# equinor/gordo

Measured on AMD Instinct MI355X. Metric: machines built/hour (1000-model config), higher is better.
Workload: dtype bf16; 1 GPU; global_batch=125, machines_per_gpu=125, seq_len=144, rows=4320, n_tags=50, epochs=5, parallelism=fleet-dp1 (RCCL shard, grouped MFMA packs per rank)

## Files before the change

### gordo_amd/ops/__init__.py

```python
from .api import (
    ACT_LINEAR,
    ACT_TANH,
    ACT_RELU,
    ACT_SIGMOID,
    act_code,
    hip_available,
    grouped_linear_fwd,
    act_l1_bwd,
    grouped_linear_bwd_data,
    grouped_linear_wgrad,
    grouped_gemm_acc,
    mse_bwd,
    adam_step,
    loss_bwd,
    optimizer_step,
    masked_copy,
    segment_table,
    lstm_pointwise_fwd,
    lstm_seq_fwd,
    lstm_seq_fwd_v3,
    lstm_seq_fwd_v2,
    lstm_seq_bwd,
    lstm_seq_bwd_v2,
    last_scan_launch,
    last_scan_activation,
    lstm_act_scan_available,
    last_wgrad_launch,
    lstm_seq_bwd_v3,
    lstm_seq_available,
    lstm_v4_available,
    lstm_seq_fwd_fused,
    lstm_seq_bwd_fused,
    lstm_seq_bwd_fused_out,
    lstm_seq_bwd_v3_out,
    anomaly_score,
    trail_min_max,
    grouped_linear_wgrad_hprev,
    window_gather,
    grouped_wgrad_xh,
    windowed_quantile,
    row_quantile,
    lstm_pointwise_bwd,
)

__all__ = [
    "ACT_LINEAR",
    "ACT_TANH",
    "ACT_RELU",
    "ACT_SIGMOID",
    "act_code",
    "hip_available",
    "grouped_linear_fwd",
    "act_l1_bwd",
    "grouped_linear_bwd_data",
    "grouped_linear_wgrad",
    "grouped_gemm_acc",
    "mse_bwd",
    "adam_step",
    "loss_bwd",
    "optimizer_step",
    "masked_copy",
    "segment_table",
    "lstm_pointwise_fwd",
    "lstm_seq_fwd",
    "lstm_seq_fwd_v3",
    "lstm_seq_fwd_v2",
    "lstm_seq_bwd",
    "lstm_seq_bwd_v2",
    "last_scan_launch",
    "last_scan_activation",
    "lstm_act_scan_available",
    "last_wgrad_launch",
    "lstm_seq_bwd_v3",
    "trail_min_max",
    "grouped_linear_wgrad_hprev",
    "window_gather",
    "grouped_wgrad_xh",
    "windowed_quantile",
    "row_quantile",
    "lstm_seq_available",
    "lstm_v4_available",
    "lstm_seq_fwd_fused",
    "lstm_seq_bwd_fused",
    "lstm_seq_bwd_fused_out",
    "lstm_seq_bwd_v3_out",
    "anomaly_score",
    "lstm_pointwise_bwd",
]
```

### gordo_amd/ops/api.py

```python
from __future__ import annotations

from typing import Optional, Tuple

import torch

from . import reference as ref
from .reference import (
    ACT_LINEAR,
    ACT_TANH,
    ACT_RELU,
    ACT_SIGMOID,
    act_code,
)

_hip = None
_hip_err: Optional[str] = None


def _load_hip():
    global _hip, _hip_err
    if _hip is not None or _hip_err is not None:
        return _hip
    try:
        from . import _gordo_hip
# ... 168 lines not shown
    elif kind == "rmsprop":
        code = _OPT_RMSPROP
        vals = [lr, h["rho"], h["momentum"], h["epsilon"]]
    elif kind == "adagrad":
        code, vals = _OPT_ADAGRAD, [lr, h["epsilon"], 0.0, 0.0]
    elif kind == "adam":
        code = _OPT_ADAM_AMSGRAD
        vals = [lr, h["beta_1"], h["beta_2"], h["epsilon"]]
    elif kind == "adamax":
        code = _OPT_ADAMAX
        vals = [lr, h["beta_1"], h["beta_2"], h["epsilon"]]
    else:
        raise ValueError(f"Unsupported optimizer {kind!r}")
    if active is not None:
        return _require_hip().optimizer_step_masked(
            code, p, g, s0, s1, s2, [float(v) for v in vals], flag, p_lp,
            step_buf, active, segments,
        )
    return _require_hip().optimizer_step(
        code, p, g, s0, s1, s2, [float(v) for v in vals], flag, p_lp,
        step_buf,
    )


def lstm_seq_fwd(xW, Wh):
    import os as _os

    ext = _require_hip()
    G, B = xW.shape[0], xW.shape[1]
    H = xW.shape[-1] // 4
    v2_fills = H % 16 == 0 and G * ((B + 63) // 64) >= 256
    if (
        _os.environ.get("GORDO_LSTM_V1") == "1"
        or H > 64
        or v2_fills
    ):
        return ext.lstm_seq_fwd(xW, Wh)
    return ext.lstm_seq_fwd_v3(xW, Wh)


def lstm_v4_available(H: int, F: int) -> bool:
    return hip_available() and H <= 64 and H % 8 == 0 and F % 8 == 0 \
        and F <= 128


def lstm_act_scan_available(H: int, F: int) -> bool:
    import os as _os

    return (
        lstm_v4_available(H, F)
        and F >= 8
        and _os.environ.get("GORDO_LSTM_V4", "1") != "0"
        and _os.environ.get("GORDO_LSTM_PIPE", "1") != "0"
    )


def lstm_seq_fwd_fused(xseq, Wx, Wh, bias, store_aux=True, act="tanh"):
    act = act_code(act)
    if _on_gpu(xseq):
        return _require_hip().lstm_seq_fwd_fused(
            xseq, Wx, Wh, bias, bool(store_aux), act
        )
    G, B, T, F = xseq.shape
    H = Wh.shape[1]
    gates_all = ref.grouped_linear_fwd(
        xseq.reshape(G, B * T, F), Wx, bias, ACT_LINEAR
    ).view(G, B, T, 4 * H)
    h = torch.zeros(G, B, H, dtype=xseq.dtype)
    c = torch.zeros(G, B, H, dtype=torch.float32)
    hs = torch.empty(G, B, T, H, dtype=xseq.dtype)
    cs = torch.empty(G, B, T, H, dtype=torch.float32)
    ga = torch.empty(G, B, T, 4 * H, dtype=xseq.dtype)
    for t in range(T):
        gates = gates_all[:, :, t] + torch.bmm(h, Wh)
        h, c, gact = ref.lstm_pointwise_fwd(gates, c, act)
        hs[:, :, t] = h
        cs[:, :, t] = c
        ga[:, :, t] = gact
    if store_aux:
        return [hs, cs, ga]
    return [hs]


def lstm_seq_fwd_v3(xW, Wh):
    return _require_hip().lstm_seq_fwd_v3(xW, Wh)


def lstm_seq_fwd_v2(xW, Wh):
    H = xW.shape[-1] // 4
    if H % 16 != 0 or H > 64:
        raise ValueError("lstm_seq_fwd_v2 needs H % 16 == 0 and H <= 64")
    return _require_hip().lstm_seq_fwd(xW, Wh)


def lstm_seq_bwd_v2(dSeq, gacts, cs, Wh, last_only):
    H = gacts.shape[-1] // 4
    if H % 16 != 0 or H > 64:
        raise ValueError("lstm_seq_bwd_v2 needs H % 16 == 0 and H <= 64")
    return _require_hip().lstm_seq_bwd(dSeq, gacts, cs, Wh, bool(last_only))


def last_scan_launch() -> dict:
    family, rows, hf, has_dx, last_only = _require_hip().last_scan_launch()
    return {
        "family": family,
        "rows": rows,
        "hf": hf if hf > 0 else None,
        "has_dx": None if has_dx < 0 else bool(has_dx),
        "last_only": None if last_only < 0 else bool(last_only),
    }


def last_scan_activation() -> str:
    return _require_hip().last_scan_activation()


def lstm_seq_bwd(dSeq, gacts, cs, Wh, last_only, act="tanh"):
    import os as _os

    ext = _require_hip()
    act = act_code(act)
    if act != ACT_TANH:
        return ext.lstm_seq_bwd_v3(dSeq, gacts, cs, Wh, bool(last_only), act)
    G, B = gacts.shape[0], gacts.shape[1]
    H = gacts.shape[-1] // 4
    v2_fills = H % 16 == 0 and G * ((B + 63) // 64) >= 256
    if (
        _os.environ.get("GORDO_LSTM_V1") == "1"
        or H > 64
        or v2_fills
    ):
        return ext.lstm_seq_bwd(dSeq, gacts, cs, Wh, last_only)
    return ext.lstm_seq_bwd_v3(dSeq, gacts, cs, Wh, last_only)


def _lstm_seq_bwd_cpu(dSeq, gacts, cs, Wh, last_only, act):
    G, B, T, H4 = gacts.shape
    H = H4 // 4
    WhT = Wh.transpose(1, 2)
    dh_carry = torch.zeros(G, B, H, dtype=gacts.dtype)
    dc = torch.zeros(G, B, H, dtype=cs.dtype)
    dG = torch.empty_like(gacts)
    zero_c = torch.zeros_like(cs[:, :, 0])
    for t in range(T - 1, -1, -1):
        dh = dh_carry
        if not last_only:
            dh = dh + dSeq[:, :, t]
        elif t == T - 1:
            dh = dh + dSeq
        c_prev = cs[:, :, t - 1] if t > 0 else zero_c
        dg, dc = ref.lstm_pointwise_bwd(
            dh, dc, gacts[:, :, t], cs[:, :, t], c_prev, act
        )
        dG[:, :, t] = dg
        dh_carry = torch.bmm(dg, WhT)
    return dG


def lstm_seq_bwd_fused(dSeq, gacts, cs, Wh, Wx, last_only, act="tanh"):
    act = act_code(act)
    if _on_gpu(gacts):
        out = _require_hip().lstm_seq_bwd_fused(
            dSeq, gacts, cs, Wh, Wx, bool(last_only), act
        )
        return out[0], out[1]
    dG = _lstm_seq_bwd_cpu(dSeq, gacts, cs, Wh, last_only, act)
    G, B, T, H4 = gacts.shape
    dX = ref.grouped_linear_bwd_data(
        dG.view(G, B * T, H4), Wx
    ).view(G, B, T, Wx.shape[1])
    return dG, dX


def lstm_seq_bwd_v3(dSeq, gacts, cs, Wh, last_only, act="tanh"):
    act = act_code(act)
    if not _on_gpu(gacts):
        return _lstm_seq_bwd_cpu(dSeq, gacts, cs, Wh, last_only, act)
    return _require_hip().lstm_seq_bwd_v3(
        dSeq, gacts, cs, Wh, bool(last_only), act
    )


def lstm_seq_bwd_fused_out(dSeq, gacts, cs, Wh, Wx, last_only, dG, dX,
                           act="tanh"):
    _require_hip().lstm_seq_bwd_fused_out(
        dSeq, gacts, cs, Wh, Wx, bool(last_only), dG, dX, act_code(act)
    )


def lstm_seq_bwd_v3_out(dSeq, gacts, cs, Wh, last_only, dG, act="tanh"):
    _require_hip().lstm_seq_bwd_v3_out(
        dSeq, gacts, cs, Wh, bool(last_only), dG, act_code(act)
    )


def lstm_seq_available(H: int) -> bool:
    if not hip_available():
# ... 56 lines not shown
```

### gordo_amd/ops/csrc/gordo_kernels.hip

```cpp

#include <hip/hip_runtime.h>
#include <hip/hip_bf16.h>
#include <torch/extension.h>
#include <ATen/cuda/CUDAContext.h>

#include <cstdint>
#include <cstdlib>
#include <string>
#include <tuple>
#include <vector>

#define DEV_INLINE __device__ __forceinline__

using bf16 = __hip_bfloat16;

typedef __attribute__((ext_vector_type(4))) float f32x4;
typedef __attribute__((ext_vector_type(8))) short bf16x8;

constexpr int ACT_LINEAR = 0, ACT_TANH = 1, ACT_RELU = 2, ACT_SIGMOID = 3;

DEV_INLINE float fast_tanhf(float x);

DEV_INLINE float act_apply(float z, int act) {
  switch (act) {
// ... 716 lines not shown
    switch (act) {                                                          \
      case ACT_LINEAR:                                                      \
        hipLaunchKernelGGL(K<ACT_LINEAR>, __VA_ARGS__); break;              \
      case ACT_RELU:                                                        \
        hipLaunchKernelGGL(K<ACT_RELU>, __VA_ARGS__); break;                \
      case ACT_SIGMOID:                                                     \
        hipLaunchKernelGGL(K<ACT_SIGMOID>, __VA_ARGS__); break;             \
      default:                                                              \
        hipLaunchKernelGGL(K<ACT_TANH>, __VA_ARGS__); break;                \
    }                                                                       \
  } while (0)

std::vector<torch::Tensor> lstm_pointwise_fwd(torch::Tensor gates,
                                              torch::Tensor c_prev,
                                              int64_t act) {
  CHECK_GPU(gates);
  TORCH_CHECK(act >= ACT_LINEAR && act <= ACT_SIGMOID,
              "unknown LSTM cell activation code ", act);
  auto gc = to_bf16c(gates);
  auto cp = c_prev.to(torch::kFloat32).contiguous();
  int H4 = gc.size(-1);
  int H = H4 / 4;
  size_t rows = gc.numel() / H4;
  auto sizes = gc.sizes().vec();
  sizes.back() = H;
  auto h = torch::empty(sizes, gc.options());
  auto c = torch::empty(sizes, gc.options().dtype(torch::kFloat32));
  auto gact = torch::empty_like(gc);
  size_t n = rows * H;
  int blocks = (int)std::min<size_t>((n + 255) / 256, 2048);
  GORDO_CELL_ACT_LAUNCH(lstm_pw_fwd_kernel, dim3(blocks), dim3(256), 0,
                        cur_stream(), (const bf16*)gc.data_ptr(),
                        cp.data_ptr<float>(), (bf16*)h.data_ptr(),
                        c.data_ptr<float>(), (bf16*)gact.data_ptr(), rows, H);
  return {h, c, gact};
}

std::vector<torch::Tensor> lstm_pointwise_bwd(torch::Tensor dh,
                                              torch::Tensor dc_next,
                                              torch::Tensor gact,
                                              torch::Tensor c,
                                              torch::Tensor c_prev,
                                              int64_t act) {
  CHECK_GPU(dh);
  TORCH_CHECK(act >= ACT_LINEAR && act <= ACT_SIGMOID,
              "unknown LSTM cell activation code ", act);
  auto dhc = to_bf16c(dh);
  auto dcn = dc_next.to(torch::kFloat32).contiguous();
  auto gc = to_bf16c(gact);
  auto cc = c.to(torch::kFloat32).contiguous();
  auto cpc = c_prev.to(torch::kFloat32).contiguous();
  int H = dhc.size(-1);
  size_t rows = dhc.numel() / H;
  auto dgates = torch::empty_like(gc);
  auto dc_prev = torch::empty_like(cc);
  size_t n = rows * H;
  int blocks = (int)std::min<size_t>((n + 255) / 256, 2048);
  GORDO_CELL_ACT_LAUNCH(lstm_pw_bwd_kernel, dim3(blocks), dim3(256), 0,
                        cur_stream(), (const bf16*)dhc.data_ptr(),
                        dcn.data_ptr<float>(), (const bf16*)gc.data_ptr(),
                        cc.data_ptr<float>(), cpc.data_ptr<float>(),
                        (bf16*)dgates.data_ptr(), dc_prev.data_ptr<float>(),
                        rows, H);
  return {dgates, dc_prev};
}
#undef GORDO_CELL_ACT_LAUNCH

}

namespace gordo_anomaly {
std::vector<torch::Tensor> anomaly_score(
    torch::Tensor out, torch::Tensor y, torch::Tensor scale,
    torch::Tensor minv, c10::optional<torch::Tensor> feat_thr,
    double agg_thr);
}

namespace gordo_lstm {
std::vector<torch::Tensor> lstm_seq_fwd(torch::Tensor xW, torch::Tensor Wh);
std::vector<torch::Tensor> lstm_seq_fwd_fused(torch::Tensor xseq,
                                              torch::Tensor Wx,
                                              torch::Tensor Wh,
                                              torch::Tensor bias,
                                              bool store_aux, int64_t act);
std::vector<torch::Tensor> lstm_seq_fwd_v3(torch::Tensor xW, torch::Tensor Wh);
torch::Tensor lstm_seq_bwd_v3(torch::Tensor dSeq, torch::Tensor gacts,
                              torch::Tensor cs, torch::Tensor Wh,
                              bool last_only, int64_t act);
std::vector<torch::Tensor> lstm_seq_bwd_fused(
    torch::Tensor dSeq, torch::Tensor gacts, torch::Tensor cs,
    torch::Tensor Wh, torch::Tensor Wx, bool last_only, int64_t act);
torch::Tensor lstm_seq_bwd(torch::Tensor dSeq, torch::Tensor gacts,
                           torch::Tensor cs, torch::Tensor Wh,
                           bool last_only);
void lstm_seq_bwd_fused_out(torch::Tensor dSeq, torch::Tensor gacts,
                            torch::Tensor cs, torch::Tensor Wh,
                            torch::Tensor Wx, bool last_only,
                            torch::Tensor dG, torch::Tensor dX, int64_t act);
void lstm_seq_bwd_v3_out(torch::Tensor dSeq, torch::Tensor gacts,
                         torch::Tensor cs, torch::Tensor Wh, bool last_only,
                         torch::Tensor dG, int64_t act);
std::tuple<std::string, int, int, int, int> last_scan_launch();
std::string last_scan_activation();
}

namespace gordo_thresholds {
torch::Tensor trail_min_max(torch::Tensor X, int64_t w);
torch::Tensor windowed_quantile(torch::Tensor X, int64_t w, double q);
torch::Tensor row_quantile(torch::Tensor X, double q);
}

namespace gordo_train {
std::vector<torch::Tensor> loss_bwd(torch::Tensor Y, torch::Tensor T,
                                    int64_t kind, int64_t real_f,
                                    double delta, bool want_grad);
void optimizer_step(int64_t kind, torch::Tensor p, torch::Tensor g,
                    c10::optional<torch::Tensor> s0,
                    c10::optional<torch::Tensor> s1,
                    c10::optional<torch::Tensor> s2,
                    std::vector<double> hyper, bool flag,
                    c10::optional<torch::Tensor> plp,
                    torch::Tensor step_buf);
}

namespace gordo_masked {
void optimizer_step_masked(int64_t kind, torch::Tensor p, torch::Tensor g,
                           c10::optional<torch::Tensor> s0,
                           c10::optional<torch::Tensor> s1,
                           c10::optional<torch::Tensor> s2,
                           std::vector<double> hyper, bool flag,
                           c10::optional<torch::Tensor> plp,
                           torch::Tensor step_buf, torch::Tensor active,
                           torch::Tensor table);
void masked_copy(torch::Tensor dst, torch::Tensor src, torch::Tensor mask,
                 torch::Tensor table, c10::optional<torch::Tensor> dst_lp);
}

PYBIND11_MODULE(TORCH_EXTENSION_NAME, mod) {
  mod.def("optimizer_step_masked", &gordo_masked::optimizer_step_masked,
          "optimizer step (every kind, plain Adam = 0) over the models "
          "with active[g] != 0 only");
  mod.def("masked_copy", &gordo_masked::masked_copy, py::arg("dst"),
          py::arg("src"), py::arg("mask"), py::arg("table"),
          py::arg("dst_lp") = py::none(),
          "copy the slices of the models with mask[g] != 0 (+ bf16 "
          "mirror)");
  mod.def("loss_bwd", &gordo_train::loss_bwd,
          "fused per-model loss (mse/mae/huber/logcosh) + grad + "
          "accuracy count, one pass over (Y, T)");
  mod.def("optimizer_step", &gordo_train::optimizer_step,
          "fused SGD/RMSprop/Adagrad/Adam-amsgrad/Adamax + bf16 mirror "
          "refresh");
  mod.def("trail_min_max", &gordo_thresholds::trail_min_max,
          "rolling(w).min().max() per row (K10)");
  mod.def("windowed_quantile", &gordo_thresholds::windowed_quantile,
          "rolling(w).quantile(q) per row — q=0.5 is the smm smoothing "
          "(K11)");
  mod.def("row_quantile", &gordo_thresholds::row_quantile,
          "NaN-dropping linear-interpolated quantile per row (K12)");
  mod.def("anomaly_score", &gordo_anomaly::anomaly_score,
          "fused DiffBased anomaly scoring (serving hot path)");
  mod.def("lstm_seq_bwd_v3", &gordo_lstm::lstm_seq_bwd_v3, py::arg("dSeq"),
          py::arg("gacts"), py::arg("cs"), py::arg("Wh"),
          py::arg("last_only"), py::arg("act") = (int64_t)ACT_TANH,
          "pipelined fused LSTM backward scan (GORDO_LSTM_V3 opt-in)");
  mod.def("lstm_seq_fwd_v3", &gordo_lstm::lstm_seq_fwd_v3,
          "pipelined fused LSTM forward scan (GORDO_LSTM_V3 opt-in)");
  mod.def("lstm_seq_fwd", &gordo_lstm::lstm_seq_fwd,
          "fused LSTM forward sequence scan (Wh resident in LDS)");
  mod.def("lstm_seq_fwd_fused", &gordo_lstm::lstm_seq_fwd_fused,
          py::arg("xseq"), py::arg("Wx"), py::arg("Wh"), py::arg("bias"),
          py::arg("store_aux"), py::arg("act") = (int64_t)ACT_TANH,
          "v4 scan with the x-side gate GEMM fused in (halves fwd "
          "HBM traffic); store_aux=false skips cs/gacts (inference)");
  mod.def("lstm_seq_bwd", &gordo_lstm::lstm_seq_bwd,
          "fused LSTM backward (BPTT) sequence scan");
  mod.def("lstm_seq_bwd_fused", &gordo_lstm::lstm_seq_bwd_fused,
          py::arg("dSeq"), py::arg("gacts"), py::arg("cs"), py::arg("Wh"),
          py::arg("Wx"), py::arg("last_only"),
          py::arg("act") = (int64_t)ACT_TANH,
          "v5 reverse scan with dSeq = dG@Wx^T fused in");
  mod.def("lstm_seq_bwd_fused_out", &gordo_lstm::lstm_seq_bwd_fused_out,
          py::arg("dSeq"), py::arg("gacts"), py::arg("cs"), py::arg("Wh"),
          py::arg("Wx"), py::arg("last_only"), py::arg("dG"), py::arg("dX"),
          py::arg("act") = (int64_t)ACT_TANH,
          "lstm_seq_bwd_fused into caller-provided dG, dX");
  mod.def("last_scan_activation", &gordo_lstm::last_scan_activation,
          "cell activation name of this thread's last scan-kernel launch");
  mod.def("last_scan_launch", &gordo_lstm::last_scan_launch,
          "(family, rows, hf, has_dx, last_only) of this thread's last "
          "scan-kernel launch");
  mod.def("lstm_seq_bwd_v3_out", &gordo_lstm::lstm_seq_bwd_v3_out,
          py::arg("dSeq"), py::arg("gacts"), py::arg("cs"), py::arg("Wh"),
          py::arg("last_only"), py::arg("dG"),
          py::arg("act") = (int64_t)ACT_TANH,
          "lstm_seq_bwd_v3 into a caller-provided dG");
  mod.def("grouped_linear_fwd", &grouped_linear_fwd,
          "Y = act(X@W + b) per group (MFMA)");
  mod.def("grouped_linear_bwd_data", &grouped_linear_bwd_data,
          "dX = dZ@W^T per group (MFMA)");
  mod.def("grouped_linear_wgrad", &grouped_linear_wgrad,
          "dW = X^T@dZ, db = colsum(dZ) per group (MFMA)");
  mod.def("grouped_linear_wgrad_hprev", &grouped_linear_wgrad_hprev,
          "dWh = h_prev^T@dG with in-kernel t-1 shift (no concat)");
  mod.def("last_wgrad_launch", &last_wgrad_launch,
          "(family, chunks, mstep) of this thread's last weight-grad "
          "launch");
  mod.def("grouped_wgrad_xh", &grouped_wgrad_xh,
          "combined {dWx, dWh, db} — dZ staged once for both");
  mod.def("window_gather", &window_gather,
          "K7 sliding-window featurizer: [G,N,F] -> [G,B,T,F]");
  mod.def("grouped_gemm_acc", &grouped_gemm_acc, "C += A@B per group (MFMA)");
  mod.def("act_l1_bwd", &act_l1_bwd, "fused activation+L1 backward");
  mod.def("mse_bwd", &mse_bwd, py::arg("Y"), py::arg("T"),
          py::arg("real_n") = -1,
          "fused per-model MSE loss + grad (real_n: divisor when the "
          "feature dim is zero-padded)");
  mod.def("adam_step", &adam_step, "fused Adam + bf16 mirror refresh");
  mod.def("lstm_pointwise_fwd", &lstm_pointwise_fwd, py::arg("gates"),
          py::arg("c_prev"), py::arg("act") = (int64_t)ACT_TANH,
          "LSTM cell fwd");
  mod.def("lstm_pointwise_bwd", &lstm_pointwise_bwd, py::arg("dh"),
          py::arg("dc_next"), py::arg("gact"), py::arg("c"),
          py::arg("c_prev"), py::arg("act") = (int64_t)ACT_TANH,
          "LSTM cell bwd");
}
```

### gordo_amd/ops/csrc/lstm_seq.hip

```cpp

#include <hip/hip_runtime.h>
#include <hip/hip_bf16.h>
#include <torch/extension.h>
#include <ATen/cuda/CUDAContext.h>

#include <string>
#include <tuple>
#include <type_traits>
#include <vector>

#define DEV_INLINE __device__ __forceinline__

using bf16 = __hip_bfloat16;
typedef __attribute__((ext_vector_type(4))) float f32x4;
typedef __attribute__((ext_vector_type(8))) short bf16x8;

DEV_INLINE float lbf2f(bf16 v) { return __bfloat162float(v); }
DEV_INLINE unsigned short bf16_bits(bf16 v) {
  return __builtin_bit_cast(unsigned short, v);
}
DEV_INLINE bf16 bits_bf16(unsigned short b) {
  return __builtin_bit_cast(bf16, b);
}
DEV_INLINE bf16 lf2bf(float v) { return __float2bfloat16(v); }
// ... 1481 lines not shown
              &hxS[(fm * 16 + l15) * LDKc + kk + kslot * 8]);
          #pragma unroll
          for (int fn = 0; fn < 4; ++fn) {
            int col = wcol0 + fn * 16 + l15;
            bf16x8 b = *reinterpret_cast<const bf16x8*>(
                &WT[(size_t)min(col, H4 - 1) * LDKc + kk + kslot * 8]);
            acc[fm][fn] = __builtin_amdgcn_mfma_f32_16x16x32_bf16(
                a, b, acc[fm][fn], 0, 0, 0);
          }
        }
      }
      #pragma unroll
      for (int fm = 0; fm < FM; ++fm) {
        #pragma unroll
        for (int fn = 0; fn < 4; ++fn) {
          int col = wcol0 + fn * 16 + l15;
          if (col >= H4) continue;
          float bv = lbf2f(bS[col]);
          #pragma unroll
          for (int r = 0; r < 4; ++r) {
            int row = fm * 16 + kslot * 4 + r;
            put_gate(&gS[row * ldg + col], acc[fm][fn][r] + bv);
          }
        }
      }
    }
    __syncthreads();

    const int nx = ROWS * (F / 8);
    if (t + 1 < T) {
      #pragma unroll
      for (int s = 0; s < NPF; ++s) {
        int i = tid + s * 256;
        if (i < nx) {
          int row = i / (F / 8), f8 = i % (F / 8);
          bf16x8 v = {};
          if (row < rows_here)
            v = *reinterpret_cast<const bf16x8*>(
                &xg[((size_t)row * T + (t + 1)) * F + f8 * 8]);
          xpf[s] = v;
        }
      }
    }

    for (int e = tid; e < ROWS * H; e += 256) {
      int row = e / H, hh = e % H;
      const gate_t* grow = &gS[row * ldg];
      float i_g = sigmoidf_(get_gate(&grow[hh]));
      float f_g = sigmoidf_(get_gate(&grow[H + hh]));
      float g_g = cell_act_<ACT>(get_gate(&grow[2 * H + hh]));
      float o_g = sigmoidf_(get_gate(&grow[3 * H + hh]));
      float cc = f_g * cS[row * H + hh] + i_g * g_g;
      float hv = o_g * cell_act_<ACT>(cc);
      cS[row * H + hh] = cc;
      hxS[row * LDKc + hh] = lf2bf(hv);
      if (row < rows_here) {
        size_t base = ((size_t)row * T + t) * H + hh;
        hsg[base] = lf2bf(hv);
        if (STORE_AUX) {
          csg[base] = cc;
          size_t gbase = ((size_t)row * T + t) * H4;
          gag[gbase + hh] = lf2bf(i_g);
          gag[gbase + H + hh] = lf2bf(f_g);
          gag[gbase + 2 * H + hh] = lf2bf(g_g);
          gag[gbase + 3 * H + hh] = lf2bf(o_g);
        }
      }
    }
    if (t + 1 < T) {
      #pragma unroll
      for (int s = 0; s < NPF; ++s) {
        int i = tid + s * 256;
        if (i < nx) {
          int row = i / (F / 8), f8 = i % (F / 8);
          *reinterpret_cast<bf16x8*>(
              &hxS[row * LDKc + H + f8 * 8]) = xpf[s];
        }
      }
    }
    __syncthreads();
  }
}

namespace gordo_lstm {

struct ScanLaunch {
  const char* family = "";
  int rows = 0;
  int hf = 0;
  int has_dx = -1;
  int last_only = -1;
};
thread_local ScanLaunch g_last_launch;
thread_local const char* g_last_act = "tanh";

inline const char* act_name(int act) {
  switch (act) {
    case CELL_LINEAR: return "linear";
    case CELL_RELU: return "relu";
    case CELL_SIGMOID: return "sigmoid";
    default: return "tanh";
  }
}

inline void check_act(int64_t act) {
  TORCH_CHECK(act >= CELL_LINEAR && act <= CELL_SIGMOID,
              "unknown LSTM cell activation code ", act);
}

inline void note_launch(const char* family, int rows, int hf = 0,
                        int has_dx = -1, int last_only = -1,
                        int act = CELL_TANH) {
  g_last_launch = ScanLaunch{family, rows, hf, has_dx, last_only};
  g_last_act = act_name(act);
}

std::string last_scan_activation() { return std::string(g_last_act); }

std::tuple<std::string, int, int, int, int> last_scan_launch() {
  const ScanLaunch& l = g_last_launch;
  return {std::string(l.family), l.rows, l.hf, l.has_dx, l.last_only};
}

inline int pad_ldg(int h4) { return ((h4 + 31) & ~31) + 8; }

inline int pick_rows(int G, int B) {
  if (const char* e = getenv("GORDO_LSTM_ROWS")) {
    int r = atoi(e);
    if (r == 16 || r == 32 || r == 64) return r;
  }
  if (G * ((B + 63) / 64) >= 512) return 64;
  if (G * ((B + 31) / 32) >= 512) return 32;
  return 16;
}

inline bool big_ok(int H) { return H > 64 && H <= 256 && H % 8 == 0; }

inline size_t big_lds(int rows, int H, int ldg, int Kp) {
  int LDH = Kp + 8;
  return (size_t)rows * LDH * 2 + (size_t)rows * ldg * 2 +
         (size_t)rows * H * 4;
}

inline int pick_rows_big(int B, int H, int ldg, int Kp) {
  if (B >= 48 && big_lds(64, H, ldg, Kp) <= 160 * 1024) return 64;
  return 32;
}

std::vector<torch::Tensor> lstm_seq_fwd_big(torch::Tensor xW,
                                            torch::Tensor Wh) {
  TORCH_CHECK(xW.is_cuda() && xW.dim() == 4, "xW must be [G,B,T,4H] on GPU");
  auto xc = xW.to(torch::kBFloat16).contiguous();
  auto Whc = Wh.to(torch::kBFloat16).contiguous();
  int G = xc.size(0), B = xc.size(1), T = xc.size(2), H4 = xc.size(3);
  int H = H4 / 4;
  TORCH_CHECK(big_ok(H), "lstm_seq_fwd_big needs 64 < H <= 256, H % 8 == 0");
  int Kp = (H + 31) & ~31;
  int ldg = pad_ldg(H4);
  auto WhT = torch::zeros({G, H4, Kp},
                          Whc.options().dtype(torch::kBFloat16));
  WhT.narrow(2, 0, H).copy_(Whc.transpose(1, 2));
  WhT = WhT.contiguous();
  auto hs = torch::empty({G, B, T, H}, xc.options());
  auto cs = torch::empty({G, B, T, H}, xc.options().dtype(torch::kFloat32));
  auto gacts = torch::empty({G, B, T, H4}, xc.options());
  int rows = pick_rows_big(B, H, ldg, Kp);
  size_t lds = big_lds(rows, H, ldg, Kp);
  TORCH_CHECK(lds <= 160 * 1024, "LDS budget exceeded (big fwd)");
  int blocks = G * ((B + rows - 1) / rows);
  auto stream = at::cuda::getCurrentCUDAStream().stream();
  note_launch("fwd_big", rows);
  if (rows == 64)
    hipLaunchKernelGGL(lstm_seq_fwd_big_kernel<64>, dim3(blocks), dim3(256),
                       lds, stream, (const bf16*)xc.data_ptr(),
                       (const bf16*)WhT.data_ptr(), (bf16*)hs.data_ptr(),
                       cs.data_ptr<float>(), (bf16*)gacts.data_ptr(), B, T, H,
                       ldg, Kp);
  else
    hipLaunchKernelGGL(lstm_seq_fwd_big_kernel<32>, dim3(blocks), dim3(256),
                       lds, stream, (const bf16*)xc.data_ptr(),
                       (const bf16*)WhT.data_ptr(), (bf16*)hs.data_ptr(),
                       cs.data_ptr<float>(), (bf16*)gacts.data_ptr(), B, T, H,
                       ldg, Kp);
  return {hs, cs, gacts};
}

torch::Tensor lstm_seq_bwd_big(torch::Tensor dSeq, torch::Tensor gacts,
                               torch::Tensor cs, torch::Tensor Wh,
                               bool last_only) {
  TORCH_CHECK(gacts.is_cuda() && gacts.dim() == 4, "gacts must be [G,B,T,4H]");
  auto dc = dSeq.to(torch::kBFloat16).contiguous();
  auto gc = gacts.to(torch::kBFloat16).contiguous();
  auto ccs = cs.to(torch::kFloat32).contiguous();
  auto Whc = Wh.to(torch::kBFloat16).contiguous();
  int G = gc.size(0), B = gc.size(1), T = gc.size(2), H4 = gc.size(3);
  int H = H4 / 4;
  TORCH_CHECK(big_ok(H), "lstm_seq_bwd_big needs 64 < H <= 256, H % 8 == 0");
  int Kp = (H + 31) & ~31;
  int ldg = pad_ldg(H4);
  auto dG = torch::empty_like(gc);
  int rows = pick_rows_big(B, H, ldg, Kp);
  size_t lds = big_lds(rows, H, ldg, Kp);
  TORCH_CHECK(lds <= 160 * 1024, "LDS budget exceeded (big bwd)");
  int blocks = G * ((B + rows - 1) / rows);
  auto stream = at::cuda::getCurrentCUDAStream().stream();
  note_launch("bwd_big", rows);
  if (rows == 64)
    hipLaunchKernelGGL(lstm_seq_bwd_big_kernel<64>, dim3(blocks), dim3(256),
                       lds, stream, (const bf16*)dc.data_ptr(),
                       (const bf16*)gc.data_ptr(), ccs.data_ptr<float>(),
                       (const bf16*)Whc.data_ptr(), (bf16*)dG.data_ptr(), B,
                       T, H, ldg, last_only ? 1 : 0);
  else
    hipLaunchKernelGGL(lstm_seq_bwd_big_kernel<32>, dim3(blocks), dim3(256),
                       lds, stream, (const bf16*)dc.data_ptr(),
                       (const bf16*)gc.data_ptr(), ccs.data_ptr<float>(),
                       (const bf16*)Whc.data_ptr(), (bf16*)dG.data_ptr(), B,
                       T, H, ldg, last_only ? 1 : 0);
  return dG;
}

inline bool v4_ok(int H, int F) {
  return H <= 64 && H % 8 == 0 && F % 8 == 0 && F <= 128;
}

std::vector<torch::Tensor> lstm_seq_fwd_fused(torch::Tensor xseq,
                                              torch::Tensor Wx,
                                              torch::Tensor Wh,
                                              torch::Tensor bias,
                                              bool store_aux, int64_t act) {
  TORCH_CHECK(xseq.is_cuda() && xseq.dim() == 4,
              "xseq must be [G,B,T,F] on GPU");
  check_act(act);
  auto xc = xseq.to(torch::kBFloat16).contiguous();
  auto Wxc = Wx.to(torch::kBFloat16);
  auto Whc = Wh.to(torch::kBFloat16);
  auto bc = bias.to(torch::kBFloat16).contiguous();
  int G = xc.size(0), B = xc.size(1), T = xc.size(2), F = xc.size(3);
  int H = Whc.size(1), H4 = 4 * H;
  TORCH_CHECK(v4_ok(H, F), "lstm_seq_fwd_fused geometry unsupported");
  int Kc = H + F;
  int LDKc = ((Kc + 31) & ~31) + 8;
  int ldg = pad_ldg(H4);
  auto Wcat = torch::cat({Whc, Wxc}, 1).transpose(1, 2).contiguous();
  auto hs = torch::empty({G, B, T, H}, xc.options());
  auto cs = store_aux
                ? torch::empty({G, B, T, H},
                               xc.options().dtype(torch::kFloat32))
                : torch::empty({1}, xc.options().dtype(torch::kFloat32));
  auto gacts = store_aux ? torch::empty({G, B, T, H4}, xc.options())
                         : torch::empty({1}, xc.options());
  int rows = pick_rows(G, B);
  const size_t gate_bytes = act == CELL_TANH ? 2 : 4;
  auto lds_for = [&](int r) {
    return (size_t)H4 * LDKc * 2 + (size_t)r * LDKc * 2 +
           (size_t)r * ldg * gate_bytes + (size_t)ldg * 2 +
           (size_t)r * H * 4;
  };
  while (rows > 16 && lds_for(rows) > 160 * 1024) rows /= 2;
  size_t lds = lds_for(rows);
  TORCH_CHECK(lds <= 160 * 1024, "LDS budget exceeded (v4 fwd)");
  int blocks = G * ((B + rows - 1) / rows);
  auto stream = at::cuda::getCurrentCUDAStream().stream();
  auto xp = (const bf16*)xc.data_ptr();
  auto wp = (const bf16*)Wcat.data_ptr();
  auto bp = (const bf16*)bc.data_ptr();
  auto hp = (bf16*)hs.data_ptr();
  auto cp = cs.data_ptr<float>();
  auto gp = (bf16*)gacts.data_ptr();
  #define V4_LAUNCH(R, S, A)                                            \
    hipLaunchKernelGGL((lstm_seq_fwd_v4_kernel<R, S, A>), dim3(blocks), \
                       dim3(256), lds, stream, xp, wp, bp, hp, cp, gp,  \
                       B, T, H, F, ldg)
  #define V4_ROWS(S, A)                                                 \
    do {                                                                \
      if (rows == 64) V4_LAUNCH(64, S, A);                              \
      else if (rows == 32) V4_LAUNCH(32, S, A);                         \
      else V4_LAUNCH(16, S, A);                                         \
    } while (0)
  #define V4_AUX(A)                                                     \
    do {                                                                \
      if (store_aux) V4_ROWS(true, A);                                  \
      else V4_ROWS(false, A);                                           \
    } while (0)
  note_launch("fwd_v4", rows, 0, -1, -1, (int)act);
  switch ((int)act) {
    case CELL_LINEAR: V4_AUX(CELL_LINEAR); break;
    case CELL_RELU: V4_AUX(CELL_RELU); break;
    case CELL_SIGMOID: V4_AUX(CELL_SIGMOID); break;
    default: V4_AUX(CELL_TANH); break;
  }
  #undef V4_AUX
  #undef V4_ROWS
  #undef V4_LAUNCH
  if (store_aux) return {hs, cs, gacts};
  return {hs};
}

std::vector<torch::Tensor> lstm_seq_fwd(torch::Tensor xW, torch::Tensor Wh) {
  TORCH_CHECK(xW.is_cuda() && xW.dim() == 4, "xW must be [G,B,T,4H] on GPU");
  if (xW.size(3) / 4 > 64) return lstm_seq_fwd_big(xW, Wh);
  auto xc = xW.to(torch::kBFloat16).contiguous();
  auto Whc = Wh.to(torch::kBFloat16).contiguous();
  int G = xc.size(0), B = xc.size(1), T = xc.size(2), H4 = xc.size(3);
  int H = H4 / 4;
  TORCH_CHECK(H <= 64, "lstm_seq_fwd supports H <= 64");
  int ldg = pad_ldg(H4);
  auto hs = torch::empty({G, B, T, H}, xc.options());
  auto cs = torch::empty({G, B, T, H}, xc.options().dtype(torch::kFloat32));
  auto gacts = torch::empty({G, B, T, H4}, xc.options());
  int rows = pick_rows(G, B);
  size_t lds = (size_t)H4 * LDK * 2 + (size_t)rows * LDK * 2 +
               (size_t)rows * ldg * 2 + (size_t)rows * H * 4;
  TORCH_CHECK(lds <= 160 * 1024, "LDS budget exceeded");
  int blocks = G * ((B + rows - 1) / rows);
  auto stream = at::cuda::getCurrentCUDAStream().stream();
  if (H % 16 == 0) {
    int blocks2 = G * ((B + 63) / 64);
    size_t lds2 = (size_t)H4 * LDK * 2 + (size_t)4 * 16 * LDK * 2;
    auto xp = (const bf16*)xc.data_ptr();
    auto wp = (const bf16*)Whc.data_ptr();
    auto hp = (bf16*)hs.data_ptr();
    auto cp = cs.data_ptr<float>();
    auto gp = (bf16*)gacts.data_ptr();
    note_launch("fwd_v2", 64, H / 16);
    switch (H / 16) {
      case 1: hipLaunchKernelGGL(lstm_seq_fwd_v2_kernel<1>, dim3(blocks2),
                                 dim3(256), lds2, stream, xp, wp, hp, cp, gp,
                                 B, T); break;
      case 2: hipLaunchKernelGGL(lstm_seq_fwd_v2_kernel<2>, dim3(blocks2),
                                 dim3(256), lds2, stream, xp, wp, hp, cp, gp,
                                 B, T); break;
      case 3: hipLaunchKernelGGL(lstm_seq_fwd_v2_kernel<3>, dim3(blocks2),
                                 dim3(256), lds2, stream, xp, wp, hp, cp, gp,
                                 B, T); break;
      default: hipLaunchKernelGGL(lstm_seq_fwd_v2_kernel<4>, dim3(blocks2),
                                 dim3(256), lds2, stream, xp, wp, hp, cp, gp,
                                 B, T); break;
    }
    return {hs, cs, gacts};
  }
  note_launch("fwd_v1", rows);
  if (rows == 64)
    hipLaunchKernelGGL(lstm_seq_fwd_kernel<64>, dim3(blocks), dim3(256), lds,
                       stream, (const bf16*)xc.data_ptr(),
                       (const bf16*)Whc.data_ptr(), (bf16*)hs.data_ptr(),
                       cs.data_ptr<float>(), (bf16*)gacts.data_ptr(), B, T, H,
                       ldg);
  else if (rows == 32)
    hipLaunchKernelGGL(lstm_seq_fwd_kernel<32>, dim3(blocks), dim3(256), lds,
                       stream, (const bf16*)xc.data_ptr(),
                       (const bf16*)Whc.data_ptr(), (bf16*)hs.data_ptr(),
                       cs.data_ptr<float>(), (bf16*)gacts.data_ptr(), B, T, H,
                       ldg);
  else
    hipLaunchKernelGGL(lstm_seq_fwd_kernel<16>, dim3(blocks), dim3(256), lds,
                       stream, (const bf16*)xc.data_ptr(),
                       (const bf16*)Whc.data_ptr(), (bf16*)hs.data_ptr(),
                       cs.data_ptr<float>(), (bf16*)gacts.data_ptr(), B, T, H,
                       ldg);
  return {hs, cs, gacts};
}

std::vector<torch::Tensor> lstm_seq_fwd_v3(torch::Tensor xW,
                                            torch::Tensor Wh) {
  TORCH_CHECK(xW.is_cuda() && xW.dim() == 4, "xW must be [G,B,T,4H] on GPU");
  if (xW.size(3) / 4 > 64) return lstm_seq_fwd_big(xW, Wh);
  auto xc = xW.to(torch::kBFloat16).contiguous();
  auto Whc = Wh.to(torch::kBFloat16).contiguous();
  int G = xc.size(0), B = xc.size(1), T = xc.size(2), H4 = xc.size(3);
  int H = H4 / 4;
  TORCH_CHECK(H <= 64, "lstm_seq_fwd_v3 supports H <= 64");
  int ldg = pad_ldg(H4);
  auto hs = torch::empty({G, B, T, H}, xc.options());
  auto cs = torch::empty({G, B, T, H}, xc.options().dtype(torch::kFloat32));
  auto gacts = torch::empty({G, B, T, H4}, xc.options());
  int rows = pick_rows(G, B);
  size_t lds = (size_t)H4 * LDK * 2 + (size_t)rows * LDK * 2 +
               (size_t)rows * ldg * 2 + (size_t)rows * H * 4;
// ... 325 lines not shown
```

Measured before the change: 92360 machines/hour.

## Add pipelined LSTM forward kernel with x prefetch, vectorized stores, in-kernel weight staging

Adds a new fused LSTM forward scan kernel that prefetches the next timestep's x rows into registers while the current step computes. Per-step outputs (h, c, gate activations) are staged in LDS and written with 16-byte vector stores instead of scalar ones. When the weights are already contiguous bf16, it builds the transposed [Wh;Wx] image inside the kernel, which skips the host-side cat/transpose/contiguous. It also adds an out-parameter entry point. The kernel is on by default when the alignment and LDS budget checks pass. The cost is an extra LDS buffer for gate activations and higher register pressure.

```diff
diff --git a/gordo_amd/ops/__init__.py b/gordo_amd/ops/__init__.py
--- a/gordo_amd/ops/__init__.py
+++ b/gordo_amd/ops/__init__.py
@@ -24,12 +24,15 @@
     lstm_seq_bwd_v2,
     last_scan_launch,
     last_scan_activation,
+    last_scan_stores,
+    last_scan_weight_staging,
     lstm_act_scan_available,
     last_wgrad_launch,
     lstm_seq_bwd_v3,
     lstm_seq_available,
     lstm_v4_available,
     lstm_seq_fwd_fused,
+    lstm_seq_fwd_fused_out,
     lstm_seq_bwd_fused,
     lstm_seq_bwd_fused_out,
     lstm_seq_bwd_v3_out,
@@ -69,6 +72,8 @@
     "lstm_seq_bwd_v2",
     "last_scan_launch",
     "last_scan_activation",
+    "last_scan_stores",
+    "last_scan_weight_staging",
     "lstm_act_scan_available",
     "last_wgrad_launch",
     "lstm_seq_bwd_v3",
@@ -81,6 +86,7 @@
     "lstm_seq_available",
     "lstm_v4_available",
     "lstm_seq_fwd_fused",
+    "lstm_seq_fwd_fused_out",
     "lstm_seq_bwd_fused",
     "lstm_seq_bwd_fused_out",
     "lstm_seq_bwd_v3_out",
diff --git a/gordo_amd/ops/api.py b/gordo_amd/ops/api.py
--- a/gordo_amd/ops/api.py
+++ b/gordo_amd/ops/api.py
@@ -274,6 +274,13 @@
     return [hs]
 
 
+def lstm_seq_fwd_fused_out(xseq, Wx, Wh, bias, store_aux, hs, cs=None,
+                           gacts=None, act="tanh"):
+    _require_hip().lstm_seq_fwd_fused_out(
+        xseq, Wx, Wh, bias, bool(store_aux), hs, cs, gacts, act_code(act)
+    )
+
+
 def lstm_seq_fwd_v3(xW, Wh):
     return _require_hip().lstm_seq_fwd_v3(xW, Wh)
 
@@ -305,6 +312,14 @@
 
 def last_scan_activation() -> str:
     return _require_hip().last_scan_activation()
+
+
+def last_scan_stores() -> str:
+    return _require_hip().last_scan_stores()
+
+
+def last_scan_weight_staging() -> str:
+    return _require_hip().last_scan_weight_staging()
 
 
 def lstm_seq_bwd(dSeq, gacts, cs, Wh, last_only, act="tanh"):
diff --git a/gordo_amd/ops/csrc/gordo_kernels.hip b/gordo_amd/ops/csrc/gordo_kernels.hip
--- a/gordo_amd/ops/csrc/gordo_kernels.hip
+++ b/gordo_amd/ops/csrc/gordo_kernels.hip
@@ -822,6 +822,11 @@
                                               torch::Tensor Wh,
                                               torch::Tensor bias,
                                               bool store_aux, int64_t act);
+void lstm_seq_fwd_fused_out(torch::Tensor xseq, torch::Tensor Wx,
+                            torch::Tensor Wh, torch::Tensor bias,
+                            bool store_aux, torch::Tensor hs,
+                            c10::optional<torch::Tensor> cs,
+                            c10::optional<torch::Tensor> gacts, int64_t act);
 std::vector<torch::Tensor> lstm_seq_fwd_v3(torch::Tensor xW, torch::Tensor Wh);
 torch::Tensor lstm_seq_bwd_v3(torch::Tensor dSeq, torch::Tensor gacts,
                               torch::Tensor cs, torch::Tensor Wh,
@@ -841,6 +846,8 @@
                          torch::Tensor dG, int64_t act);
 std::tuple<std::string, int, int, int, int> last_scan_launch();
 std::string last_scan_activation();
+std::string last_scan_stores();
+std::string last_scan_weight_staging();
 }
 
 namespace gordo_thresholds {
@@ -912,6 +919,17 @@
           py::arg("store_aux"), py::arg("act") = (int64_t)ACT_TANH,
           "v4 scan with the x-side gate GEMM fused in (halves fwd "
           "HBM traffic); store_aux=false skips cs/gacts (inference)");
+  mod.def("lstm_seq_fwd_fused_out", &gordo_lstm::lstm_seq_fwd_fused_out,
+          py::arg("xseq"), py::arg("Wx"), py::arg("Wh"), py::arg("bias"),
+          py::arg("store_aux"), py::arg("hs"), py::arg("cs") = py::none(),
+          py::arg("gacts") = py::none(), py::arg("act") = (int64_t)ACT_TANH,
+          "lstm_seq_fwd_fused into caller-provided hs, cs, gacts");
+  mod.def("last_scan_stores", &gordo_lstm::last_scan_stores,
+          "\"vec16\" / \"scalar\": how this thread's last scan launch "
+          "stored its per-step outputs");
+  mod.def("last_scan_weight_staging", &gordo_lstm::last_scan_weight_staging,
+          "\"kernel\" / \"host\": who built the last v4 forward's "
+          "[Wh ; Wx]^T image");
   mod.def("lstm_seq_bwd", &gordo_lstm::lstm_seq_bwd,
           "fused LSTM backward (BPTT) sequence scan");
   mod.def("lstm_seq_bwd_fused", &gordo_lstm::lstm_seq_bwd_fused,
diff --git a/gordo_amd/ops/csrc/lstm_seq.hip b/gordo_amd/ops/csrc/lstm_seq.hip
--- a/gordo_amd/ops/csrc/lstm_seq.hip
+++ b/gordo_amd/ops/csrc/lstm_seq.hip
@@ -1587,6 +1587,242 @@
   }
 }
 
+template <int ROWS, bool STORE_AUX, int ACT>
+__global__ __launch_bounds__(256) void lstm_seq_fwd_pipe_kernel(
+    const bf16* __restrict__ xseq,
+    const bf16* __restrict__ WcatT,
+    const bf16* __restrict__ Wh,
+    const bf16* __restrict__ Wx,
+    const bf16* __restrict__ bias,
+    bf16* __restrict__ hs, float* __restrict__ cs,
+    bf16* __restrict__ gacts, int B, int T, int H, int F, int ldg) {
+  extern __shared__ __attribute__((aligned(16))) char smem[];
+  const int H4 = 4 * H;
+  const int Kc = H + F;
+  const int LDKc = ((Kc + 31) & ~31) + 8;
+  bf16* WT = reinterpret_cast<bf16*>(smem);
+  bf16* hxS = WT + (size_t)H4 * LDKc;
+  using gate_t = gate_tile_t<ACT>;
+  gate_t* gS = reinterpret_cast<gate_t*>(hxS + (size_t)ROWS * LDKc);
+  bf16* bS = reinterpret_cast<bf16*>(gS + (size_t)ROWS * ldg);
+  float* cS = reinterpret_cast<float*>(bS + ldg);
+  bf16* gaS = reinterpret_cast<bf16*>(cS + (size_t)ROWS * H);
+
+  const int nb = (B + ROWS - 1) / ROWS;
+  const int g = blockIdx.x / nb;
+  const int r0 = (blockIdx.x % nb) * ROWS;
+  const int tid = threadIdx.x;
+  const int lane = tid & 63;
+  const int wid = __builtin_amdgcn_readfirstlane(tid >> 6);
+  const int l15 = lane & 15;
+  const int kslot = lane >> 4;
+
+  const bf16* xg = xseq + ((size_t)g * B + r0) * T * F;
+  bf16* hsg = hs + ((size_t)g * B + r0) * T * H;
+  float* csg = cs + ((size_t)g * B + r0) * T * H;
+  bf16* gag = gacts + ((size_t)g * B + r0) * T * H4;
+  const int rows_here = min(ROWS, B - r0);
+
+  constexpr int NPF = ROWS / 16;
+  const int F8 = F / 8;
+  const int nx = ROWS * F8;
+  const bf16* x_src[NPF];
+  int x_dst[NPF];
+  bool x_live[NPF];
+  bf16x8 xpf[NPF];
+  #pragma unroll
+  for (int s = 0; s < NPF; ++s) {
+    int i = tid + s * 256;
+    int ic = min(i, nx - 1);
+    int row = ic / F8, f8 = ic % F8;
+    x_src[s] = xg + (size_t)min(row, rows_here - 1) * T * F + f8 * 8;
+    x_dst[s] = (i < nx) ? row * LDKc + H + f8 * 8 : -1;
+    x_live[s] = row < rows_here;
+  }
+  auto load_x = [&](int tt) {
+    tt = min(tt, T - 1);
+    #pragma unroll
+    for (int s = 0; s < NPF; ++s)
+      xpf[s] = *reinterpret_cast<const bf16x8*>(x_src[s] + (size_t)tt * F);
+  };
+  auto write_x = [&]() {
+    #pragma unroll
+    for (int s = 0; s < NPF; ++s) {
+      bf16x8 z = {};
+      if (x_dst[s] >= 0)
+        *reinterpret_cast<bf16x8*>(&hxS[x_dst[s]]) = x_live[s] ? xpf[s] : z;
+    }
+  };
+  load_x(0);
+
+  const int CPR = (H / 8) * (STORE_AUX ? 7 : 1);
+  constexpr int NST = (ROWS * (STORE_AUX ? 56 : 8) + 255) / 256;
+  const int total = ROWS * CPR;
+  int st_src[NST];
+  unsigned st_ok = 0;
+  char* st_dst[NST];
+  int st_str[NST];
+  #pragma unroll
+  for (int s = 0; s < NST; ++s) {
+    int c = min(tid + s * 256, total - 1);
+    int row = c / CPR, j = c % CPR;
+    bool ok = tid + s * 256 < total && row < rows_here;
+    size_t rt = (size_t)row * T;
+    const char* src;
+    if (!STORE_AUX || j < H / 8) {
+      src = reinterpret_cast<const char*>(hxS + row * LDKc + j * 8);
+      st_dst[s] = reinterpret_cast<char*>(hsg + rt * H + j * 8);
+      st_str[s] = H * 2;
+    } else if (j < H / 8 + H / 4) {
+      int jj = j - H / 8;
+      src = reinterpret_cast<const char*>(cS + row * H + jj * 4);
+      st_dst[s] = reinterpret_cast<char*>(csg + rt * H + jj * 4);
+      st_str[s] = H * 4;
+    } else {
+      int jj = j - H / 8 - H / 4;
+      src = reinterpret_cast<const char*>(gaS + row * H4 + jj * 8);
+      st_dst[s] = reinterpret_cast<char*>(gag + rt * H4 + jj * 8);
+      st_str[s] = H4 * 2;
+    }
+    st_src[s] = (int)(src - smem);
+    st_ok |= ok ? (1u << s) : 0u;
+  }
+
+  constexpr int NE = ROWS / 4;
+  int e_rc[NE];
+  #pragma unroll
+  for (int k = 0; k < NE; ++k) {
+    int e = tid + k * 256;
+    e_rc[k] = (e < ROWS * H) ? ((e / H) << 8) | (e % H) : -1;
+  }
+
+  if (WcatT != nullptr) {
+    const bf16* WTg = WcatT + (size_t)g * H4 * Kc;
+    for (int i = tid; i < H4 * LDKc; i += 256) {
+      int n = i / LDKc, k = i % LDKc;
+      WT[i] = (k < Kc) ? WTg[(size_t)n * Kc + k] : lf2bf(0.f);
+    }
+  } else {
+    const bf16* Whg = Wh + (size_t)g * H * H4;
+    const bf16* Wxg = Wx + (size_t)g * F * H4;
+    for (int i = tid; i < (LDKc / 2) * H4; i += 256) {
+      int k = (i / H4) * 2, n = i % H4;
+      unsigned int lo = 0, hi = 0;
+      if (k < Kc) {
+        const bf16* src = (k < H) ? Whg + (size_t)k * H4 + n
+                                  : Wxg + (size_t)(k - H) * H4 + n;
+        lo = bf16_bits(src[0]);
+        hi = bf16_bits(src[H4]);
+      }
+      *reinterpret_cast<unsigned int*>(&WT[(size_t)n * LDKc + k]) =
+          lo | (hi << 16);
+    }
+  }
+  for (int i = tid; i < ldg; i += 256)
+    bS[i] = (i < H4) ? bias[(size_t)g * H4 + i] : lf2bf(0.f);
+  for (int i = tid; i < ROWS * LDKc; i += 256) {
+    int k = i % LDKc;
+    if (k < H || k >= H + F) hxS[i] = lf2bf(0.f);
+  }
+  for (int i = tid; i < ROWS * H; i += 256) cS[i] = 0.f;
+  write_x();
+  load_x(1);
+  __syncthreads();
+
+  constexpr int FM = ROWS / 16;
+  const int nfw = (H4 / 16 - wid + 3) / 4;
+  const bf16* wtp = WT + (size_t)(wid * 16 + l15) * LDKc + kslot * 8;
+  const bf16* hxp = hxS + l15 * LDKc + kslot * 8;
+
+  auto mfma_phase = [&](auto nf_c) {
+    constexpr int NFW = decltype(nf_c)::value;
+    f32x4 acc[FM][NFW] = {};
+    for (int kk = 0; kk < Kc; kk += 32) {
+      bf16x8 b[NFW];
+      #pragma unroll
+      for (int fn = 0; fn < NFW; ++fn)
+        b[fn] = *reinterpret_cast<const bf16x8*>(
+            &wtp[(size_t)fn * 64 * LDKc + kk]);
+      #pragma unroll
+      for (int fm = 0; fm < FM; ++fm) {
+        bf16x8 a = *reinterpret_cast<const bf16x8*>(
+            &hxp[fm * 16 * LDKc + kk]);
+        #pragma unroll
+        for (int fn = 0; fn < NFW; ++fn)
+          acc[fm][fn] = __builtin_amdgcn_mfma_f32_16x16x32_bf16(
+              a, b[fn], acc[fm][fn], 0, 0, 0);
+      }
+    }
+    #pragma unroll
+    for (int fn = 0; fn < NFW; ++fn) {
+      int col = (wid + 4 * fn) * 16 + l15;
+      float bv = lbf2f(bS[col]);
+      #pragma unroll
+      for (int fm = 0; fm < FM; ++fm) {
+        #pragma unroll
+        for (int r = 0; r < 4; ++r) {
+          int row = fm * 16 + kslot * 4 + r;
+          put_gate(&gS[row * ldg + col], acc[fm][fn][r] + bv);
+        }
+      }
+    }
+  };
+
+  for (int t = 0; t < T; ++t) {
+    switch (nfw) {
+      case 4: mfma_phase(std::integral_constant<int, 4>{}); break;
+      case 3: mfma_phase(std::integral_constant<int, 3>{}); break;
+      case 2: mfma_phase(std::integral_constant<int, 2>{}); break;
+      case 1: mfma_phase(std::integral_constant<int, 1>{}); break;
+      default: break;
+    }
+    __syncthreads();
+
+    write_x();
+    load_x(t + 2);
+
+    #pragma unroll
+    for (int k = 0; k < NE; ++k) {
+      if (e_rc[k] >= 0) {
+        const int row = e_rc[k] >> 8, hh = e_rc[k] & 255;
+        const gate_t* grow = &gS[row * ldg + hh];
+        float* cp = &cS[tid + k * 256];
+        float i_g = sigmoidf_(get_gate(&grow[0]));
+        float f_g = sigmoidf_(get_gate(&grow[H]));
+        float g_g = cell_act_<ACT>(get_gate(&grow[2 * H]));
+        float o_g = sigmoidf_(get_gate(&grow[3 * H]));
+        float cc = f_g * *cp + i_g * g_g;
+        float hv = o_g * cell_act_<ACT>(cc);
+        *cp = cc;
+        hxS[row * LDKc + hh] = lf2bf(hv);
+        if (STORE_AUX) {
+          bf16* ap = &gaS[row * H4 + hh];
+          ap[0] = lf2bf(i_g);
+          ap[H] = lf2bf(f_g);
+          ap[2 * H] = lf2bf(g_g);
+          ap[3 * H] = lf2bf(o_g);
+        }
+      }
+    }
+    __syncthreads();
+
+    #pragma unroll
+    for (int s0 = 0; s0 < NST; s0 += 4) {
+      constexpr int NB = NST < 4 ? NST : 4;
+      u32x4 sv[NB];
+      #pragma unroll
+      for (int s = s0; s < s0 + NB && s < NST; ++s)
+        sv[s - s0] = *reinterpret_cast<const u32x4*>(smem + st_src[s]);
+      #pragma unroll
+      for (int s = s0; s < s0 + NB && s < NST; ++s) {
+        if (st_ok & (1u << s))
+          *reinterpret_cast<u32x4*>(st_dst[s] + (size_t)t * st_str[s]) =
+              sv[s - s0];
+      }
+    }
+  }
+}
+
 namespace gordo_lstm {
 
 struct ScanLaunch {
@@ -1598,6 +1834,8 @@
 };
 thread_local ScanLaunch g_last_launch;
 thread_local const char* g_last_act = "tanh";
+thread_local const char* g_last_stores = "scalar";
+thread_local const char* g_last_wstage = "host";
 
 inline const char* act_name(int act) {
   switch (act) {
@@ -1618,9 +1856,15 @@
                         int act = CELL_TANH) {
   g_last_launch = ScanLaunch{family, rows, hf, has_dx, last_only};
   g_last_act = act_name(act);
+  g_last_stores = "scalar";
+  g_last_wstage = "host";
 }
 
 std::string last_scan_activation() { return std::string(g_last_act); }
+std::string last_scan_stores() { return std::string(g_last_stores); }
+std::string last_scan_weight_staging() {
+  return std::string(g_last_wstage);
+}
 
 std::tuple<std::string, int, int, int, int> last_scan_launch() {
   const ScanLaunch& l = g_last_launch;
@@ -1729,32 +1973,50 @@
   return H <= 64 && H % 8 == 0 && F % 8 == 0 && F <= 128;
 }
 
-std::vector<torch::Tensor> lstm_seq_fwd_fused(torch::Tensor xseq,
-                                              torch::Tensor Wx,
-                                              torch::Tensor Wh,
-                                              torch::Tensor bias,
-                                              bool store_aux, int64_t act) {
+inline void check_fwd_out(const torch::Tensor& out, const torch::Tensor& like,
+                          torch::ScalarType dtype,
+                          std::vector<int64_t> shape, const char* what) {
+  TORCH_CHECK(out.is_cuda() && out.scalar_type() == dtype &&
+                  out.is_contiguous() && out.sizes().vec() == shape &&
+                  out.device() == like.device(),
+              what, " must be a contiguous tensor of the output shape and "
+              "dtype on the inputs' device");
+}
+
+inline bool aligned16(const torch::Tensor& t) {
+  return reinterpret_cast<uintptr_t>(t.data_ptr()) % 16 == 0;
+}
+
+std::vector<torch::Tensor> lstm_seq_fwd_fused_impl(
+    torch::Tensor xseq, torch::Tensor Wx, torch::Tensor Wh,
+    torch::Tensor bias, bool store_aux, c10::optional<torch::Tensor> hs_out,
+    c10::optional<torch::Tensor> cs_out,
+    c10::optional<torch::Tensor> gacts_out, int64_t act) {
   TORCH_CHECK(xseq.is_cuda() && xseq.dim() == 4,
               "xseq must be [G,B,T,F] on GPU");
   check_act(act);
   auto xc = xseq.to(torch::kBFloat16).contiguous();
-  auto Wxc = Wx.to(torch::kBFloat16);
-  auto Whc = Wh.to(torch::kBFloat16);
   auto bc = bias.to(torch::kBFloat16).contiguous();
   int G = xc.size(0), B = xc.size(1), T = xc.size(2), F = xc.size(3);
-  int H = Whc.size(1), H4 = 4 * H;
+  int H = Wh.size(1), H4 = 4 * H;
   TORCH_CHECK(v4_ok(H, F), "lstm_seq_fwd_fused geometry unsupported");
   int Kc = H + F;
   int LDKc = ((Kc + 31) & ~31) + 8;
   int ldg = pad_ldg(H4);
-  auto Wcat = torch::cat({Whc, Wxc}, 1).transpose(1, 2).contiguous();
-  auto hs = torch::empty({G, B, T, H}, xc.options());
-  auto cs = store_aux
-                ? torch::empty({G, B, T, H},
-                               xc.options().dtype(torch::kFloat32))
-                : torch::empty({1}, xc.options().dtype(torch::kFloat32));
-  auto gacts = store_aux ? torch::empty({G, B, T, H4}, xc.options())
-                         : torch::empty({1}, xc.options());
+  auto f32 = xc.options().dtype(torch::kFloat32);
+  if (hs_out)
+    check_fwd_out(*hs_out, xc, torch::kBFloat16, {G, B, T, H}, "hs");
+  if (store_aux && cs_out)
+    check_fwd_out(*cs_out, xc, torch::kFloat32, {G, B, T, H}, "cs");
+  if (store_aux && gacts_out)
+    check_fwd_out(*gacts_out, xc, torch::kBFloat16, {G, B, T, H4}, "gacts");
+  auto hs = hs_out ? *hs_out : torch::empty({G, B, T, H}, xc.options());
+  auto cs = !store_aux ? torch::empty({1}, f32)
+            : cs_out   ? *cs_out
+                       : torch::empty({G, B, T, H}, f32);
+  auto gacts = !store_aux   ? torch::empty({1}, xc.options())
+               : gacts_out  ? *gacts_out
+                            : torch::empty({G, B, T, H4}, xc.options());
   int rows = pick_rows(G, B);
   const size_t gate_bytes = act == CELL_TANH ? 2 : 4;
   auto lds_for = [&](int r) {
@@ -1765,18 +2027,47 @@
   while (rows > 16 && lds_for(rows) > 160 * 1024) rows /= 2;
   size_t lds = lds_for(rows);
   TORCH_CHECK(lds <= 160 * 1024, "LDS budget exceeded (v4 fwd)");
+  const size_t lds_pipe = lds + (store_aux ? (size_t)rows * H4 * 2 : 0);
+  const char* sw = getenv("GORDO_LSTM_FWD_PIPE");
+  bool pipe = !(sw && atoi(sw) == 0) && lds_pipe <= 160 * 1024 &&
+              aligned16(xc) && aligned16(hs) &&
+              (!store_aux || (aligned16(cs) && aligned16(gacts)));
+  bool native_w = pipe && Wh.scalar_type() == torch::kBFloat16 &&
+                  Wx.scalar_type() == torch::kBFloat16 &&
+                  Wh.is_contiguous() && Wx.is_contiguous() &&
+                  Wh.device() == xc.device() && Wx.device() == xc.device();
+  TORCH_CHECK(Wh.dim() == 3 && Wx.dim() == 3 && Wh.size(0) == G &&
+                  Wx.size(0) == G && Wx.size(1) == F && Wh.size(2) == H4 &&
+                  Wx.size(2) == H4 && bc.numel() == (int64_t)G * H4,
+              "lstm_seq_fwd_fused: Wx [G,F,4H], Wh [G,H,4H], bias [G,4H]");
+  torch::Tensor Wcat;
+  if (!native_w) {
+    Wcat = torch::cat({Wh.to(torch::kBFloat16), Wx.to(torch::kBFloat16)}, 1)
+               .transpose(1, 2)
+               .contiguous();
+  }
   int blocks = G * ((B + rows - 1) / rows);
   auto stream = at::cuda::getCurrentCUDAStream().stream();
   auto xp = (const bf16*)xc.data_ptr();
-  auto wp = (const bf16*)Wcat.data_ptr();
+  auto wp = native_w ? (const bf16*)nullptr : (const bf16*)Wcat.data_ptr();
+  auto whp = native_w ? (const bf16*)Wh.data_ptr() : (const bf16*)nullptr;
+  auto wxp = native_w ? (const bf16*)Wx.data_ptr() : (const bf16*)nullptr;
   auto bp = (const bf16*)bc.data_ptr();
   auto hp = (bf16*)hs.data_ptr();
   auto cp = cs.data_ptr<float>();
   auto gp = (bf16*)gacts.data_ptr();
-  #define V4_LAUNCH(R, S, A)                                            \
-    hipLaunchKernelGGL((lstm_seq_fwd_v4_kernel<R, S, A>), dim3(blocks), \
-                       dim3(256), lds, stream, xp, wp, bp, hp, cp, gp,  \
-                       B, T, H, F, ldg)
+  #define V4_LAUNCH(R, S, A)                                             \
+    do {                                                                 \
+      if (pipe)                                                          \
+        hipLaunchKernelGGL((lstm_seq_fwd_pipe_kernel<R, S, A>),          \
+                           dim3(blocks), dim3(256), lds_pipe, stream,    \
+                           xp, wp, whp, wxp, bp, hp, cp, gp, B, T, H, F, \
+                           ldg);                                         \
+      else                                                               \
+        hipLaunchKernelGGL((lstm_seq_fwd_v4_kernel<R, S, A>),            \
+                           dim3(blocks), dim3(256), lds, stream, xp, wp, \
+                           bp, hp, cp, gp, B, T, H, F, ldg);             \
+    } while (0)
   #define V4_ROWS(S, A)                                                 \
     do {                                                                \
       if (rows == 64) V4_LAUNCH(64, S, A);                              \
@@ -1789,6 +2080,8 @@
       else V4_ROWS(false, A);                                           \
     } while (0)
   note_launch("fwd_v4", rows, 0, -1, -1, (int)act);
+  g_last_stores = pipe ? "vec16" : "scalar";
+  g_last_wstage = native_w ? "kernel" : "host";
   switch ((int)act) {
     case CELL_LINEAR: V4_AUX(CELL_LINEAR); break;
     case CELL_RELU: V4_AUX(CELL_RELU); break;
@@ -1800,6 +2093,27 @@
   #undef V4_LAUNCH
   if (store_aux) return {hs, cs, gacts};
   return {hs};
+}
+
+std::vector<torch::Tensor> lstm_seq_fwd_fused(torch::Tensor xseq,
+                                              torch::Tensor Wx,
+                                              torch::Tensor Wh,
+                                              torch::Tensor bias,
+                                              bool store_aux, int64_t act) {
+  return lstm_seq_fwd_fused_impl(xseq, Wx, Wh, bias, store_aux,
+                                 c10::nullopt, c10::nullopt, c10::nullopt,
+                                 act);
+}
+
+void lstm_seq_fwd_fused_out(torch::Tensor xseq, torch::Tensor Wx,
+                            torch::Tensor Wh, torch::Tensor bias,
+                            bool store_aux, torch::Tensor hs,
+                            c10::optional<torch::Tensor> cs,
+                            c10::optional<torch::Tensor> gacts,
+                            int64_t act) {
+  TORCH_CHECK(!store_aux || (cs && gacts),
+              "lstm_seq_fwd_fused_out: store_aux needs cs and gacts");
+  lstm_seq_fwd_fused_impl(xseq, Wx, Wh, bias, store_aux, hs, cs, gacts, act);
 }
 
 std::vector<torch::Tensor> lstm_seq_fwd(torch::Tensor xW, torch::Tensor Wh) {
```

After: 90450 machines/hour. 2.1% lower.
